# cfnptr/garden

Measured on AMD Instinct MI355X. Metric: entity culls/sec at 10M entities; visible-set bit-match vs CPU ref, higher is better.
Workload: dtype f32; 1 GPU; cfg3: 10M entities, frustum + Hi-Z occlusion vs synthetic 4096^2 depth pyramid (rebuilt per frame); depth=walls, entities_per_gpu=10000000, entities_total=10000000, scaling_mode=weak: 10000000 entities per GPU, hiz=4096x4096, prewarm_frames=2800

## Files before the change

### garden_amd/csrc/gv_cull.hip

```cpp
#include "gv_device.hpp"

#include <type_traits>

namespace gv {

template <typename F>
__host__ __device__ __forceinline__ void with_mapping(uint32_t mapping, F&& f)
{
    switch (mapping) {
    case kMapExact: f(std::integral_constant<uint32_t, kMapExact>{}); break;
    case kMapSpeculate: f(std::integral_constant<uint32_t, kMapSpeculate>{}); break;
    default: f(std::integral_constant<uint32_t, kMapGeneral>{}); break;
    }
}
template <typename F>
__host__ __device__ __forceinline__ void with_variant(bool hiz, uint32_t mapping, F&& f)
{
    if (hiz)
        with_mapping(mapping, [&](auto map) { f(std::true_type{}, map); });
    else
        with_mapping(mapping, [&](auto map) { f(std::false_type{}, map); });
}

__device__ __forceinline__ bool block_behind_planes(const float4 lo, const float4 hi, const float (&planes)[6][4],
                                                    uint32_t plane_count, const float (&cam)[3], uint32_t max_depth)
{
    const float mag = fmaxf(fabsf(lo.x), fabsf(hi.x)) + fmaxf(fabsf(lo.y), fabsf(hi.y)) + fmaxf(fabsf(lo.z), fabsf(hi.z)) +
                      fabsf(cam[0]) + fabsf(cam[1]) + fabsf(cam[2]);
    const float margin = 0.01f + 4e-5f * (float)(max_depth + 1u) * mag;
    bool behind = false;
#pragma unroll
    for (uint32_t p = 0; p < 6; p++)
        if (p < plane_count) {
            const float nx = planes[p][0], ny = planes[p][1], nz = planes[p][2];
            const float x = (nx >= 0.0f ? hi.x : lo.x) - cam[0];
            const float y = (ny >= 0.0f ? hi.y : lo.y) - cam[1];
            const float z = (nz >= 0.0f ? hi.z : lo.z) - cam[2];
            const float d = fmaf(nx, x, fmaf(ny, y, fmaf(nz, z, planes[p][3])));
            behind = behind || (d < -fmaf(4e-5f, fabsf(planes[p][3]), margin));
        }
    return behind;
}

typedef const CullArgs __attribute__((address_space(4))) * ConstCullArgs;
__device__ __forceinline__ void reload_cull_args(CullArgs& out)
{
    ConstCullArgs kernarg = (ConstCullArgs)__builtin_amdgcn_kernarg_segment_ptr();
    asm volatile("" : "+s"(kernarg));
    __builtin_memcpy(&out, kernarg, sizeof(out));
}

template <bool HIZ, uint32_t MAP, bool RELOAD = false, bool HOT = false>
__device__ __forceinline__ void cull_block(const CullArgs& args0, uint32_t lb, uint32_t* wave_count)
{
    static_assert(!HOT || MAP == kMapExact, "the sphere stream exists for exactly paired pools only");
    CullArgs stage1;
    if (RELOAD)
        reload_cull_args(stage1);
    const CullArgs& args = RELOAD ? stage1 : args0;
    uint32_t tid = threadIdx.x;
    if (RELOAD)
        asm volatile("" : "+v"(tid));
    const uint32_t i = lb * kCullBlock + tid;
    const uint32_t lane = tid & 63u, wave = tid >> 6;
    bool visible = false;
    Corners c;
    if (HOT && i < args.mesh.count) {
        const float4 h = stream_load(&args.mesh.hot[i]);
        uint32_t where = kSphereOutside;
        if (!(h.w < 0.0f)) {
            const float tx = h.x - args.view.cam[0], ty = h.y - args.view.cam[1], tz = h.z - args.view.cam[2];
            where = classify_sphere(tx, ty, tz, sphere_reach(h.w, tx, ty, tz), args.view.planes, args.view.plane_count);
        }
        visible = where == kSphereInside;
        if (where == kSphereUndecided || (HIZ && visible)) {
            Mat34 m;
            float4 box_a;
            float2 box_b;
            visible = prepare_model<MAP>(args.mesh, args.xf, args.view.cam, i, m, box_a, box_b) &&
                      settle<HIZ>(where, m, box_a, box_b, args.view.planes, args.view.plane_count, c);
        }
    } else if (!HOT && i < args.mesh.count) {
        Mat34 m;
        float4 box_a;
        float2 box_b;
        uint32_t where = kSphereOutside;
        if (prepare_model<MAP>(args.mesh, args.xf, args.view.cam, i, m, box_a, box_b))
            where = classify_sphere(m, box_a, box_b, args.view.planes, args.view.plane_count);
        visible = settle<HIZ>(where, m, box_a, box_b, args.view.planes, args.view.plane_count, c);
    }
    if (HIZ && visible) {
        CullArgs stage2;
        if (RELOAD)
            reload_cull_args(stage2);
        const CullArgs& a2 = RELOAD ? stage2 : args0;
        visible = !hiz_occluded(a2.hiz, a2.view.vp, c);
    }
    CullArgs stage3;
    if (RELOAD)
        reload_cull_args(stage3);
    const CullArgs& out_args = RELOAD ? stage3 : args0;
    if (i < out_args.mesh.count && out_args.view.write_is_visible)
        out_args.out.is_visible[i] = visible ? 1 : 0;
    __shared__ unsigned long long wave_word[kCullBlock / 64];
    const unsigned long long word = __ballot(visible);
    if (lane == 0) {
        wave_word[wave] = word;
        wave_count[wave] = (uint32_t)__popcll(word);
    }
    __syncthreads();
    if (tid < kCullBlock / 64)
        out_args.out.mask[(size_t)lb * (kCullBlock / 64) + tid] = wave_word[tid];
    if (tid == 0) {
        uint32_t total = 0;
#pragma unroll
        for (uint32_t w = 0; w < kCullBlock / 64; w++)
            total += wave_count[w];
        if (total)
            atomicAdd(&out_args.out.chunk_count[lb / (kEmitChunk / kCullBlock)], total);
    }
}

template <bool HIZ, uint32_t MAP, bool HOT = false>
__global__ __launch_bounds__(kCullBlock) void cull_kernel(const CullArgs args)
{
    __shared__ uint32_t wave_count[kCullBlock / 64];
    const uint32_t lb = tile_of_workgroup(blockIdx.x, args.xcd_run);
    if (lb >= args.nblocks)
        return;
    cull_block<HIZ, MAP, false, HOT>(args, lb, wave_count);
}

template <bool HIZ, uint32_t K>
__global__ __launch_bounds__(kCullBlock) void cull_hot_kernel(const CullArgs args)
{
    static_assert(K >= 2 && K <= 16 && (kEmitChunk / kCullBlock) % K == 0, "a super-tile must not straddle an emit chunk");
    __shared__ unsigned long long words[K * (kCullBlock / 64)];
    __shared__ uint32_t wave_count[kCullBlock / 64];
    const uint32_t first = tile_of_workgroup(blockIdx.x, args.xcd_run) * K;
    if (first >= args.nblocks)
        return;
    const uint32_t tid = threadIdx.x, lane = tid & 63u, wave = tid >> 6;
    const uint32_t base = first * kCullBlock + tid;
    float4 h[K];
#pragma unroll
    for (uint32_t k = 0; k < K; k++) {
        const uint32_t i = base + k * kCullBlock;
        h[k] = i < args.mesh.count ? stream_load(&args.mesh.hot[i]) : make_float4(0.0f, 0.0f, 0.0f, kHotDropped);
    }
    uint32_t where = 0;
#pragma unroll
    for (uint32_t k = 0; k < K; k++)
        if (!(h[k].w < 0.0f)) {
            const float tx = h[k].x - args.view.cam[0], ty = h[k].y - args.view.cam[1], tz = h[k].z - args.view.cam[2];
            where |= classify_sphere(tx, ty, tz, sphere_reach(h[k].w, tx, ty, tz), args.view.planes, args.view.plane_count) << (2u * k);
        }
    uint32_t count = 0;
#pragma unroll 1
    for (uint32_t k = 0; k < K; k++) {
        const uint32_t i = base + k * kCullBlock;
        const uint32_t wk = (where >> (2u * k)) & 3u;
        bool visible = wk == kSphereInside;
        if (wk == kSphereUndecided || (HIZ && visible)) {
            CullArgs a1;
            reload_cull_args(a1);
            Mat34 m;
            float4 box_a;
            float2 box_b;
            Corners c;
            visible = prepare_model<kMapExact>(a1.mesh, a1.xf, a1.view.cam, i, m, box_a, box_b) &&
                      settle<HIZ>(wk, m, box_a, box_b, a1.view.planes, a1.view.plane_count, c);
            if (HIZ && visible) {
                CullArgs a2;
                reload_cull_args(a2);
                visible = !hiz_occluded(a2.hiz, a2.view.vp, c);
            }
        }
        CullArgs a3;
        reload_cull_args(a3);
        if (i < a3.mesh.count && a3.view.write_is_visible)
            a3.out.is_visible[i] = visible ? 1 : 0;
        const unsigned long long word = __ballot(visible);
        if (lane == 0) {
            words[k * (kCullBlock / 64) + wave] = word;
            count += (uint32_t)__popcll(word);
        }
    }
    if (lane == 0)
        wave_count[wave] = count;
    __syncthreads();
    if (tid < K * (kCullBlock / 64) && first + tid / (kCullBlock / 64) < args.nblocks)
        args.out.mask[(size_t)first * (kCullBlock / 64) + tid] = words[tid];
    if (tid == 0) {
        uint32_t total = 0;
#pragma unroll
        for (uint32_t w = 0; w < kCullBlock / 64; w++)
            total += wave_count[w];
        if (total)
            atomicAdd(&args.out.chunk_count[first / (kEmitChunk / kCullBlock)], total);
    }
}

struct BlockWindow {
    uint32_t block;
    uint32_t level;
    uint32_t origin;
    float znear;
};
__device__ __forceinline__ BlockWindow block_window(const HizDevice& hz, const ViewParams& view, const float4 lo, const float4 hi,
                                                    uint32_t max_depth, uint32_t lb)
{
    BlockWindow out{lb, 0xFFu, 0u, 0.0f};
    if (!hz.nested)
        return out;
    const float (&vp)[16] = view.vp;
    const float mag = fmaxf(fabsf(lo.x), fabsf(hi.x)) + fmaxf(fabsf(lo.y), fabsf(hi.y)) + fmaxf(fabsf(lo.z), fabsf(hi.z)) +
                      fabsf(view.cam[0]) + fabsf(view.cam[1]) + fabsf(view.cam[2]);
    const float margin = 0.01f + 4e-5f * (float)(max_depth + 1u) * mag;
    const float bx[2] = {lo.x - view.cam[0] - margin, hi.x - view.cam[0] + margin};
    const float by[2] = {lo.y - view.cam[1] - margin, hi.y - view.cam[1] + margin};
    const float bz[2] = {lo.z - view.cam[2] - margin, hi.z - view.cam[2] + margin};
    const float inf = __builtin_huge_valf();
    float nx0 = inf, nx1 = -inf, ny0 = inf, ny1 = -inf, znear = -inf, wmin = inf;
    bool bounded = true;
#pragma unroll
    for (int k = 0; k < 8; k++) {
        const float x = bx[k & 1], y = by[(k >> 1) & 1], z = bz[k >> 2];
        const float clx = fmaf(vp[0], x, fmaf(vp[4], y, fmaf(vp[8], z, vp[12])));
        const float cly = fmaf(vp[1], x, fmaf(vp[5], y, fmaf(vp[9], z, vp[13])));
        const float clz = fmaf(vp[2], x, fmaf(vp[6], y, fmaf(vp[10], z, vp[14])));
        const float clw = fmaf(vp[3], x, fmaf(vp[7], y, fmaf(vp[11], z, vp[15])));
        bounded = bounded && (clw > 0.0f);
        const float rcp = 1.0f / clw;
        const float ndx = clx * rcp, ndy = cly * rcp, ndz = clz * rcp;
        nx0 = fminf(nx0, ndx); nx1 = fmaxf(nx1, ndx);
        ny0 = fminf(ny0, ndy); ny1 = fmaxf(ny1, ndy);
        znear = fmaxf(znear, ndz);
        wmin = fminf(wmin, clw);
    }
    if (!bounded)
        return out;
    const float r = lo.w;
    const float r0 = fmaxf(fmaxf(fabsf(vp[0]), fabsf(vp[4])), fabsf(vp[8])), r1 = fmaxf(fmaxf(fabsf(vp[1]), fabsf(vp[5])), fabsf(vp[9]));
    const float r3 = fmaxf(fmaxf(fabsf(vp[3]), fabsf(vp[7])), fabsf(vp[11]));
    const float span = 2.0f * r / wmin;
    const float ext_x = 0.5f * (float)hz.width * span * fmaf(fmaxf(fabsf(nx0), fabsf(nx1)), r3, r0) + 3.0f;
    const float ext_y = 0.5f * (float)hz.height * span * fmaf(fmaxf(fabsf(ny0), fabsf(ny1)), r3, r1) + 3.0f;
    const float n_max = fmaxf(ext_x, ext_y);
    if (!(n_max < 32768.0f))
        return out;
    const uint32_t l_max = (31u - (uint32_t)__clz((int)n_max)) + 1u;
    const int W = (int)hz.width, H = (int)hz.height;
    const float umin = clamp01(fmaf(nx0, 0.5f, 0.5f)), umax = clamp01(fmaf(nx1, 0.5f, 0.5f));
    const float vmin = clamp01(fmaf(ny0, 0.5f, 0.5f)), vmax = clamp01(fmaf(ny1, 0.5f, 0.5f));
    const int ix0 = max((int)(umin * (float)W) - 1, 0), ix1 = min((int)(umax * (float)W) + 1, W - 1);
    const int iy0 = max((int)(vmin * (float)H) - 1, 0), iy1 = min((int)(vmax * (float)H) + 1, H - 1);
    uint32_t level = min(l_max, hz.mip_count - 1u);
    while (level + 1u < hz.mip_count && (((ix1 >> level) - (ix0 >> level)) > 15 || ((iy1 >> level) - (iy0 >> level)) > 15))
        level++;
    const int lw = max(W >> level, 1), lh = max(H >> level, 1);
    const int tx0 = min(ix0 >> level, lw - 1), tx1 = min(ix1 >> level, lw - 1);
    const int ty0 = min(iy0 >> level, lh - 1), ty1 = min(iy1 >> level, lh - 1);
    if (tx1 - tx0 > 15 || ty1 - ty0 > 15)
        return out;
    out.level = level | ((uint32_t)(tx1 - tx0) << 8) | ((uint32_t)(ty1 - ty0) << 12);
    out.origin = (uint32_t)tx0 | ((uint32_t)ty0 << 16);
    out.znear = fmaf(fabsf(znear), 2e-6f, znear);
    return out;
}

struct ClassifyArgs {
    BlockBounds bounds;
    HizDevice hiz;
    ViewParams view;
    unsigned long long* mask;
    uint8_t* is_visible;
    uint32_t* kept_count;
    BlockWindow* kept;
    uint8_t* kept_flag;
    uint32_t nblocks, count, max_depth;
};

__device__ __forceinline__ void write_skipped_block(const ClassifyArgs& a, uint32_t lb)
{
    uint4* words = reinterpret_cast<uint4*>(a.mask + (size_t)lb * (kCullBlock / 64));
    words[0] = make_uint4(0, 0, 0, 0);
    words[1] = make_uint4(0, 0, 0, 0);
    if (a.view.write_is_visible) {
        const uint32_t first = lb * kCullBlock, end = min(first + kCullBlock, a.count);
        for (uint32_t s = first; s < end; s++)
            a.is_visible[s] = 0;
    }
}

template <bool HIZ>
__global__ __launch_bounds__(64) void block_classify_kernel(const ClassifyArgs a)
{
    const uint32_t lb = blockIdx.x * 64u + threadIdx.x;
    bool kept = false;
    BlockWindow win{lb, 0xFFu, 0u, 0.0f};
    if (lb < a.nblocks) {
        const float4 lo = a.bounds.lo[lb], hi = a.bounds.hi[lb];
        kept = !(lo.x > hi.x || block_behind_planes(lo, hi, a.view.planes, a.view.plane_count, a.view.cam, a.max_depth));
        if (HIZ && kept)
            win = block_window(a.hiz, a.view, lo, hi, a.max_depth, lb);
        if (!HIZ || !kept)
            a.bounds.examined[lb] = kept ? 1 : 0;
        if (!kept)
            write_skipped_block(a, lb);
    }
    const unsigned long long keep = __ballot(kept);
    if (keep == 0ull)
        return;
    uint32_t base = 0;
    if (threadIdx.x == 0)
        base = atomicAdd(a.kept_count, (uint32_t)__popcll(keep));
    base = (uint32_t)__builtin_amdgcn_readfirstlane((int)base);
    if (kept)
        a.kept[base + (uint32_t)__popcll(keep & ((1ull << threadIdx.x) - 1ull))] = win;
}

__global__ __launch_bounds__(256) void block_window_kernel(const ClassifyArgs a)
{
    const uint32_t lane = threadIdx.x & 63u;
    const uint32_t waves = gridDim.x * 4u;
    const uint32_t first = (uint32_t)__builtin_amdgcn_readfirstlane((int)(blockIdx.x * 4u + (threadIdx.x >> 6)));
    BlockWindow next = a.kept[min(first, a.nblocks - 1u)];
    const uint32_t listed = *a.kept_count;
    const float inf = __builtin_huge_valf();
    for (uint32_t j = first; j < listed; j += waves) {
        const BlockWindow w = next;
        if (j + waves < listed)
            next = a.kept[j + waves];
        bool occluded = false;
        const uint32_t level = w.level & 0xFFu;
        if (level != 0xFFu) {
            const uint32_t dx = (w.level >> 8) & 15u, dy = (w.level >> 12) & 15u, tx0 = w.origin & 0xFFFFu, ty0 = w.origin >> 16;
            const uint32_t lw = max(a.hiz.width >> level, 1u);
            const uint32_t lx = lane & 15u;
            float m = inf;
            bool nan = false;
#pragma unroll
            for (uint32_t q = 0; q < 4; q++) {
                const uint32_t ly = (lane >> 4) + 4u * q;
                float t = inf;
                if (lx <= dx && ly <= dy)
                    t = hiz_min_texel(a.hiz, level, lw, tx0 + lx, ty0 + ly);
                nan = nan || t != t;
                m = fminf(m, t);
            }
#pragma unroll
            for (uint32_t d = 32; d >= 1; d >>= 1)
                m = fminf(m, __shfl_xor(m, d, 64));
            occluded = __ballot(nan) == 0ull && w.znear < m;
        }
        if (lane == 0) {
            a.kept_flag[j] = occluded ? 0 : 1;
            a.bounds.examined[w.block] = occluded ? 0 : 1;
        }
        if (occluded) {
            if (lane < kCullBlock / 64)
                a.mask[(size_t)w.block * (kCullBlock / 64) + lane] = 0ull;
            if (a.view.write_is_visible) {
                const uint32_t slot = w.block * kCullBlock + 4u * lane;
                if (slot + 3u < a.count)
                    *reinterpret_cast<uint32_t*>(a.is_visible + slot) = 0u;
                else
                    for (uint32_t s = 0; slot + s < a.count && s < 4u; s++)
                        a.is_visible[slot + s] = 0;
            }
        }
    }
}

struct CullListArgs {
    const uint32_t* kept_count;
    const BlockWindow* kept;
    const uint8_t* kept_flag;
    uint32_t* next_count;
};

template <bool HIZ, uint32_t MAP>
__global__ __launch_bounds__(kCullBlock, 8) void cull_list_kernel(const CullArgs args, const CullListArgs la)
{
    __shared__ uint32_t wave_count[kCullBlock / 64];
    uint32_t flag = la.kept_flag ? la.kept_flag[blockIdx.x] : 1u;
    uint32_t block = la.kept[blockIdx.x].block;
    const uint32_t listed = *la.kept_count;
    if (blockIdx.x == 0 && threadIdx.x == 0)
        *la.next_count = 0;
    for (uint32_t j = blockIdx.x; j < listed;) {
        if (__builtin_amdgcn_readfirstlane((int)flag)) {
            cull_block<HIZ, MAP, true>(args, (uint32_t)__builtin_amdgcn_readfirstlane((int)block), wave_count);
            __syncthreads();
        }
        j += gridDim.x;
        if (j < listed) {
            flag = la.kept_flag ? la.kept_flag[j] : 1u;
            block = la.kept[j].block;
        }
    }
}

hipError_t launch_cull_listed(const MeshMirror& mesh, const TransformMirror& xf, const HizDevice& hiz, const ViewParams& vp,
                              const ViewBuffers& out, const BlockBounds& bounds, uint32_t* kept_count, uint32_t* next_count,
                              void* kept_list, uint8_t* kept_flag, hipStream_t stream)
{
    if (mesh.count == 0)
        return hipSuccess;
    const uint32_t nblocks = (mesh.count + kCullBlock - 1) / kCullBlock;
    const bool window_test = vp.use_hiz && hiz.nested;
    ClassifyArgs c{};
    c.bounds = bounds;
    c.hiz = hiz;
    c.view = vp;
    c.mask = out.mask;
    c.is_visible = out.is_visible;
    c.kept_count = kept_count;
    c.kept = static_cast<BlockWindow*>(kept_list);
    c.kept_flag = kept_flag;
    c.nblocks = nblocks;
    c.count = mesh.count;
    c.max_depth = xf.max_depth;
    const uint32_t list_grid = (nblocks + 3u) / 4u;
    if (window_test) {
        hipLaunchKernelGGL(block_classify_kernel<true>, dim3((nblocks + 63) / 64), dim3(64), 0, stream, c);
        hipLaunchKernelGGL(block_window_kernel, dim3((list_grid + 3u) / 4u), dim3(256), 0, stream, c);
    } else {
        hipLaunchKernelGGL(block_classify_kernel<false>, dim3((nblocks + 63) / 64), dim3(64), 0, stream, c);
    }
    CullArgs a{};
    a.mesh = mesh;
    a.xf = xf;
    a.hiz = hiz;
    a.view = vp;
    a.out = out;
    a.nblocks = nblocks;
    const CullListArgs la{kept_count, static_cast<const BlockWindow*>(kept_list), window_test ? kept_flag : nullptr, next_count};
    with_variant(vp.use_hiz, mesh.mapping, [&](auto hiz, auto map) {
        hipLaunchKernelGGL((cull_list_kernel<hiz, map>), dim3(list_grid), dim3(kCullBlock), 0, stream, a, la);
    });
    return hipGetLastError();
}
size_t cull_list_entry_bytes() { return sizeof(BlockWindow); }

struct FusedEmit {
    unsigned long long* status;
    uint32_t* ticket;
    uint32_t ticket_base;
    uint32_t epoch;
};
constexpr unsigned long long kTileAggregate = 1ull << 30, kTilePrefix = 2ull << 30, kTileFlagMask = 3ull << 30, kTileCountMask = (1ull << 30) - 1ull;

template <bool HIZ, uint32_t MAP>
__global__ __launch_bounds__(kCullBlock) void cull_emit_kernel(const CullArgs args, const FusedEmit fe)
{
    __shared__ uint32_t wave_count[kCullBlock / 64];
    __shared__ uint32_t tile_s, base_s;
    __shared__ float4 stage[kCullBlock * 3];
// ... 1197 lines not shown
```

### garden_amd/csrc/gv_device.hpp

```cpp
#pragma once
#include "gv_kernels.hpp"

#include <algorithm>

#include "gv_device_math.hpp"

namespace gv {


typedef float f32x4n __attribute__((ext_vector_type(4)));
typedef float f32x2n __attribute__((ext_vector_type(2)));
__device__ __forceinline__ float4 stream_load(const float4* p)
{
    const f32x4n v = __builtin_nontemporal_load(reinterpret_cast<const f32x4n*>(p));
    return make_float4(v.x, v.y, v.z, v.w);
}
__device__ __forceinline__ float2 stream_load(const float2* p)
{
    const f32x2n v = __builtin_nontemporal_load(reinterpret_cast<const f32x2n*>(p));
    return make_float2(v.x, v.y);
}
__device__ __forceinline__ uint32_t stream_load(const uint32_t* p) { return __builtin_nontemporal_load(p); }
__device__ __forceinline__ void stream_store(float4* p, float4 v)
{
    __builtin_nontemporal_store(f32x4n{v.x, v.y, v.z, v.w}, reinterpret_cast<f32x4n*>(p));
}
__device__ __forceinline__ void stream_store(float* p, float v) { __builtin_nontemporal_store(v, p); }
__device__ __forceinline__ uint32_t stream_load(const uint8_t* p) { return __builtin_nontemporal_load(p); }

struct XfRecord {
    float4 a, b;
    float2 c;
    uint32_t flags;
};
__device__ __forceinline__ XfRecord load_xf(const TransformMirror& xf, uint32_t s)
{
    XfRecord r;
    r.a = xf.ab[s].a;
    r.b = xf.ab[s].b;
    r.c = xf.c[s];
    r.flags = xf.flags[s];
    return r;
}
__device__ __forceinline__ XfRecord gather_xf(const TransformMirror& xf, uint32_t s, bool with_flags)
{
    XfRecord r;
    r.a = xf.ab[s].a;
    r.b = xf.ab[s].b;
    r.c = xf.c[s];
    r.flags = with_flags ? xf.flags[s] : 0u;
    return r;
}
__device__ __forceinline__ XfRecord stream_xf(const TransformMirror& xf, uint32_t s)
{
    XfRecord r;
    r.a = stream_load(&xf.ab[s].a);
    r.b = stream_load(&xf.ab[s].b);
    r.c = stream_load(&xf.c[s]);
    r.flags = stream_load(&xf.flags[s]);
    return r;
}
__device__ __forceinline__ Mat34 local_model(const XfRecord& r)
{
    return calc_model(r.a.x, r.a.y, r.a.z, r.b.x, r.b.y, r.b.z, r.b.w, r.a.w, r.c.x, r.c.y);
}

__device__ __forceinline__ void model_rows(const Mat34& m, float4& w0, float4& w1, float4& w2)
{
    w0 = make_float4(m.c0x, m.c0y, m.c0z, m.c1x);
    w1 = make_float4(m.c1y, m.c1z, m.c2x, m.c2y);
    w2 = make_float4(m.c2z, m.c3x, m.c3y, m.c3z);
}
__device__ __forceinline__ Mat34 rows_model(const float4 w0, const float4 w1, const float4 w2)
{
    Mat34 m;
    m.c0x = w0.x; m.c0y = w0.y; m.c0z = w0.z;
    m.c1x = w0.w; m.c1y = w1.x; m.c1z = w1.y;
    m.c2x = w1.z; m.c2y = w1.w; m.c2z = w2.x;
    m.c3x = w2.y; m.c3y = w2.z; m.c3z = w2.w;
    return m;
}

__device__ __forceinline__ Mat34 chain_model(const TransformMirror& xf, Mat34 m, uint32_t s, uint32_t flags)
{
    if (xf.max_depth != 0 && (flags & kXfWithAncestors)) {
        uint32_t p = xf.parent[s];
        for (uint32_t d = 0; d < xf.max_depth && p != kSlotNone; d++) {
            const XfRecord pr = load_xf(xf, p);
            m = mul_affine(local_model(pr), m);
            p = xf.parent[p];
        }
    }
    return m;
}

__device__ __forceinline__ float hiz_min_texel(const HizDevice& hz, uint32_t level, uint32_t lw, uint32_t x, uint32_t y)
{
    if (level == 0)
        return hz.depth[(size_t)y * hz.width + x];
    if (level == 1 && hz.level1_virtual) {
        const float2* row0 = reinterpret_cast<const float2*>(hz.depth + (size_t)(2 * y) * hz.width + 2 * x);
        const float2* row1 = reinterpret_cast<const float2*>(hz.depth + (size_t)(2 * y + 1) * hz.width + 2 * x);
        const float2 a = *row0, b = *row1;
        float m = a.x;
        m = a.y < m ? a.y : m;
        m = b.x < m ? b.x : m;
        m = b.y < m ? b.y : m;
        return hz.rg16f ? half_to_float(half_directed(m, false)) : m;
    }
    const uint64_t at = hz.mip_offset[level] + (uint64_t)y * lw + x;
    if (hz.rg16f)
        return half_to_float(reinterpret_cast<const uint32_t*>(hz.mips)[at] & 0xFFFFu);
    return hz.mips[at].x;
}
__device__ __forceinline__ float2 hiz_pair(const HizDevice& hz, uint64_t at)
{
    if (hz.rg16f)
        return unpack_rg16f(reinterpret_cast<const uint32_t*>(hz.mips)[at]);
    return hz.mips[at];
}

__device__ __forceinline__ float clamp01(float a)
{
    return a > 0.0f ? (a < 1.0f ? a : 1.0f) : 0.0f;
}

constexpr uint32_t kHizCoarseStep = 4;

__device__ __forceinline__ bool hiz_occluded(const HizDevice& hz, const float (&vp)[16], const Corners& c)
{
    float u[8], v[8], zc[8];
    bool bounded = true;
#pragma unroll
    for (int j = 0; j < 4; j++) {
        const v2f clx = pk_fma(splat(vp[0]), c.x[j], pk_fma(splat(vp[4]), c.y[j], pk_fma(splat(vp[8]), c.z[j], splat(vp[12]))));
        const v2f cly = pk_fma(splat(vp[1]), c.x[j], pk_fma(splat(vp[5]), c.y[j], pk_fma(splat(vp[9]), c.z[j], splat(vp[13]))));
        const v2f clz = pk_fma(splat(vp[2]), c.x[j], pk_fma(splat(vp[6]), c.y[j], pk_fma(splat(vp[10]), c.z[j], splat(vp[14]))));
        const v2f clw = pk_fma(splat(vp[3]), c.x[j], pk_fma(splat(vp[7]), c.y[j], pk_fma(splat(vp[11]), c.z[j], splat(vp[15]))));
        bounded = bounded && (clw.x > 0.0f) && (clw.y > 0.0f);
        const v2f rcp = {1.0f / clw.x, 1.0f / clw.y};
        const v2f uu = pk_fma(clx * rcp, splat(0.5f), splat(0.5f));
        const v2f vv = pk_fma(cly * rcp, splat(0.5f), splat(0.5f));
        const v2f zz = clz * rcp;
        u[2 * j] = uu.x; u[2 * j + 1] = uu.y;
        v[2 * j] = vv.x; v[2 * j + 1] = vv.y;
        zc[2 * j] = zz.x; zc[2 * j + 1] = zz.y;
    }
    if (!bounded)
        return false;
    const float umin0 = fminf(fminf(fminf(u[0], u[1]), fminf(u[2], u[3])), fminf(fminf(u[4], u[5]), fminf(u[6], u[7])));
    const float umax0 = fmaxf(fmaxf(fmaxf(u[0], u[1]), fmaxf(u[2], u[3])), fmaxf(fmaxf(u[4], u[5]), fmaxf(u[6], u[7])));
    const float vmin0 = fminf(fminf(fminf(v[0], v[1]), fminf(v[2], v[3])), fminf(fminf(v[4], v[5]), fminf(v[6], v[7])));
    const float vmax0 = fmaxf(fmaxf(fmaxf(v[0], v[1]), fmaxf(v[2], v[3])), fmaxf(fmaxf(v[4], v[5]), fmaxf(v[6], v[7])));
    const float znear = fmaxf(fmaxf(fmaxf(zc[0], zc[1]), fmaxf(zc[2], zc[3])), fmaxf(fmaxf(zc[4], zc[5]), fmaxf(zc[6], zc[7])));
    float umin = umin0, umax = umax0, vmin = vmin0, vmax = vmax0;
    umin = clamp01(umin);
    umax = clamp01(umax);
    vmin = clamp01(vmin);
    vmax = clamp01(vmax);
    const int W = (int)hz.width, H = (int)hz.height;
    int ix0 = (int)(umin * (float)W), ix1 = (int)(umax * (float)W);
    int iy0 = (int)(vmin * (float)H), iy1 = (int)(vmax * (float)H);
    ix0 = min(ix0, W - 1);
    ix1 = min(ix1, W - 1);
    iy0 = min(iy0, H - 1);
    iy1 = min(iy1, H - 1);
    auto axis_level = [](int i0, int i1) -> uint32_t {
        const int n = i1 - i0;
        if (n <= 1)
            return 0u;
        const uint32_t l = 31u - (uint32_t)__clz(n);
        return ((i1 >> l) - (i0 >> l)) <= 1 ? l : l + 1u;
    };
    const uint32_t level = min(max(axis_level(ix0, ix1), axis_level(iy0, iy1)), hz.mip_count - 1u);
    if (hz.nested && level + kHizCoarseStep < hz.mip_count) {
        const uint32_t cl = level + kHizCoarseStep;
        const int cw = max((int)(hz.width >> cl), 1), ch = max((int)(hz.height >> cl), 1);
        const int cx0 = min(ix0 >> cl, cw - 1), cx1 = min(ix1 >> cl, cw - 1);
        const int cy0 = min(iy0 >> cl, ch - 1), cy1 = min(iy1 >> cl, ch - 1);
        const uint64_t coarse = hz.mip_offset[cl];
        float2 t = hiz_pair(hz, coarse + (uint64_t)cy0 * cw + cx0);
        float cmin = t.x, cmax = t.y;
        if (cx1 != cx0) {
            t = hiz_pair(hz, coarse + (uint64_t)cy0 * cw + cx1);
            cmin = fminf(cmin, t.x);
            cmax = fmaxf(cmax, t.y);
        }
        if (cy1 != cy0) {
            t = hiz_pair(hz, coarse + (uint64_t)cy1 * cw + cx0);
            cmin = fminf(cmin, t.x);
            cmax = fmaxf(cmax, t.y);
            if (cx1 != cx0) {
                t = hiz_pair(hz, coarse + (uint64_t)cy1 * cw + cx1);
                cmin = fminf(cmin, t.x);
                cmax = fmaxf(cmax, t.y);
            }
        }
        if (znear < cmin)
            return true;
        if (znear >= cmax)
            return false;
    }
    const int lw = max((int)(hz.width >> level), 1), lh = max((int)(hz.height >> level), 1);
    const int tx0 = min(ix0 >> level, lw - 1), tx1 = min(ix1 >> level, lw - 1);
    const int ty0 = min(iy0 >> level, lh - 1), ty1 = min(iy1 >> level, lh - 1);
    float zfar = hiz_min_texel(hz, level, lw, tx0, ty0);
    float a = hiz_min_texel(hz, level, lw, tx1, ty0);
    zfar = a < zfar ? a : zfar;
    a = hiz_min_texel(hz, level, lw, tx0, ty1);
    zfar = a < zfar ? a : zfar;
    a = hiz_min_texel(hz, level, lw, tx1, ty1);
    zfar = a < zfar ? a : zfar;
    return znear < zfar;
}

inline uint32_t xcd_run_for_tiles(uint32_t tiles)
{
    return tiles >= 8u * 256u * 8u ? 256u : (tiles >= 8u * 32u * 8u ? 32u : 0u);
}

__device__ __forceinline__ uint32_t tile_of_workgroup(uint32_t b, uint32_t run)
{
    if (run == 0)
        return b;
    const uint32_t xcd = b & 7u, k = b >> 3;
    return ((k / run) * 8u + xcd) * run + k % run;
}

inline uint32_t grid_for_tiles(uint32_t tiles, uint32_t run)
{
    const uint32_t group = run * 8u;
    return run ? (tiles + group - 1) / group * group : tiles;
}

struct CullArgs {
    MeshMirror mesh;
    TransformMirror xf;
    HizDevice hiz;
    ViewParams view;
    ViewBuffers out;
    uint32_t nblocks;
    uint32_t xcd_run;
};

__device__ __forceinline__ bool mesh_entry_dropped(bool candidate, const float4& a, const float2& b, uint32_t xf_flags)
{
    const bool empty = (a.w - a.x <= 0.0f) && (b.x - a.y <= 0.0f) && (b.y - a.z <= 0.0f);
    return !candidate || empty || !(xf_flags & kXfActive);
}

template <uint32_t MAP>
__device__ __forceinline__ bool prepare_model(const MeshMirror& mesh, const TransformMirror& xf, const float (&cam)[3],
                                              uint32_t i, Mat34& m, float4& ma, float2& mb)
{
    ma = stream_load(&mesh.a[i]);
    mb = stream_load(&mesh.b[i]);
    uint32_t slot = i;
    bool candidate = true;
    XfRecord r = {};
    if (MAP == kMapGeneral) {
        const uint32_t link = stream_load(&mesh.link[i]);
        slot = link & kSlotMask;
        candidate = (link & kMeshCandidate) && slot != kSlotNone;
        if (candidate)
            r = load_xf(xf, slot);
    } else {
        const bool own = i < xf.count;
        if (own) {
            if (MAP == kMapExact && xf.max_depth == 0) {
                r.a = stream_load(&xf.ab[i].a);
                r.b = stream_load(&xf.ab[i].b);
                r.c = stream_load(&xf.c[i]);
                r.flags = (uint32_t)((xf.active_bits[i >> 6] >> (i & 63u)) & 1ull) * kXfActive;
            } else {
                r = stream_xf(xf, i);
            }
        }
        if (MAP == kMapSpeculate) {
            const uint32_t link = stream_load(&mesh.link[i]);
            slot = link & kSlotMask;
            candidate = (link & kMeshCandidate) && slot != kSlotNone;
            if (candidate && !(own && slot == i))
                r = load_xf(xf, slot);
        } else {
            candidate = own;
        }
    }
    if (mesh_entry_dropped(candidate, ma, mb, r.flags))
        return false;
    const Mat34 world = chain_model(xf, local_model(r), slot, r.flags);
    m = translated(world, cam[0], cam[1], cam[2]);
    return true;
}

__device__ __forceinline__ void aabb_corners(const Mat34& m, const float4 a, const float2 b, Corners& c)
{
    aabb_corners(m, a.x, a.y, a.z, a.w, b.x, b.y, c);
}

enum : uint32_t { kSphereOutside = 0, kSphereInside = 1, kSphereUndecided = 2 };
__device__ __forceinline__ float sphere_radius(const Mat34& m, const float4 a, const float2 b)
{
    const float ax = max_nan(fabsf(a.x), fabsf(a.w)), ay = max_nan(fabsf(a.y), fabsf(b.x)), az = max_nan(fabsf(a.z), fabsf(b.y));
    return fmaf(fabsf(m.c0x) + fabsf(m.c0y) + fabsf(m.c0z), ax,
                fmaf(fabsf(m.c1x) + fabsf(m.c1y) + fabsf(m.c1z), ay, (fabsf(m.c2x) + fabsf(m.c2y) + fabsf(m.c2z)) * az));
}
__device__ __forceinline__ float sphere_reach(float r, float tx, float ty, float tz)
{
    const float mag = max_nan(max_nan(fabsf(tx), fabsf(ty)), fabsf(tz)) + r;
    return fmaf(4e-5f, mag, r) + 0.01f;
}
__device__ __forceinline__ float sphere_reach(const Mat34& m, const float4 a, const float2 b)
{
    return sphere_reach(sphere_radius(m, a, b), m.c3x, m.c3y, m.c3z);
}
__device__ __forceinline__ uint32_t classify_sphere(float tx, float ty, float tz, float reach, const float (&planes)[6][4], uint32_t plane_count)
{
    bool outside = false, decided = true;
#pragma unroll
    for (uint32_t p = 0; p < 6; p++)
        if (p < plane_count) {
            const float bound = fmaf(4e-5f, fabsf(planes[p][3]), reach);
            const float d = fmaf(planes[p][0], tx, fmaf(planes[p][1], ty, fmaf(planes[p][2], tz, planes[p][3])));
            outside = outside | (d < -bound);
            decided = decided & ((d > bound) | (d < -bound));
        }
    return outside ? kSphereOutside : (decided ? kSphereInside : kSphereUndecided);
}
__device__ __forceinline__ uint32_t classify_sphere(const Mat34& m, float reach, const float (&planes)[6][4], uint32_t plane_count)
{
    return classify_sphere(m.c3x, m.c3y, m.c3z, reach, planes, plane_count);
}
__device__ __forceinline__ uint32_t classify_sphere(const Mat34& m, const float4 a, const float2 b, const float (&planes)[6][4],
                                                    uint32_t plane_count)
{
    return classify_sphere(m, sphere_reach(m, a, b), planes, plane_count);
}

__device__ __forceinline__ float4 hot_entry(const MeshMirror& mesh, const TransformMirror& xf, uint32_t i)
{
    const float zero[3] = {0.0f, 0.0f, 0.0f};
    Mat34 m;
    float4 a;
    float2 b;
    if (!prepare_model<kMapExact>(mesh, xf, zero, i, m, a, b))
        return make_float4(0.0f, 0.0f, 0.0f, kHotDropped);
    return make_float4(m.c3x, m.c3y, m.c3z, sphere_radius(m, a, b));
}

__device__ __forceinline__ bool behind_frustum(const Corners& c, const float (&planes)[6][4], uint32_t plane_count)
{
    bool behind = false;
#pragma unroll
    for (uint32_t p = 0; p < 6; p++)
        if (p < plane_count)
            behind = behind || all_behind_plane(c, planes[p][0], planes[p][1], planes[p][2], planes[p][3]);
    return behind;
}

template <bool HIZ>
__device__ __forceinline__ bool settle(uint32_t where, const Mat34& m, const float4 a, const float2 b, const float (&planes)[6][4],
                                       uint32_t plane_count, Corners& c)
{
    bool visible = where == kSphereInside;
    if (where == kSphereUndecided) {
        aabb_corners(m, a, b, c);
        visible = !behind_frustum(c, planes, plane_count);
    } else if (HIZ && visible) {
        aabb_corners(m, a, b, c);
    }
    return visible;
}
__device__ __forceinline__ bool settle(uint32_t where, bool hiz, const Mat34& m, const float4 a, const float2 b,
                                       const float (&planes)[6][4], uint32_t plane_count, Corners& c, bool& have_corners)
{
    bool visible = where == kSphereInside;
    if (where == kSphereUndecided || (hiz && visible)) {
        if (!have_corners) {
            aabb_corners(m, a, b, c);
            have_corners = true;
        }
        if (where == kSphereUndecided)
            visible = !behind_frustum(c, planes, plane_count);
    }
    return visible;
}

__device__ __forceinline__ float record_distance(const ViewParams& view, const Mat34& m)
{
    const float tx = m.c3x + view.cam_offset[0];
    const float ty = m.c3y + view.cam_offset[1];
    const float tz = m.c3z + view.cam_offset[2];
    return view.distance_2d ? m.c3z + 1.0f : fmaf(tz, tz, fmaf(ty, ty, tx * tx));
}
__device__ __forceinline__ void put_record(const ViewParams& view, const ViewBuffers& out, size_t rank, uint32_t slot, const Mat34& m,
                                           float4* row)
{
    out.visible_idx[rank] = slot;
    out.distance_sq[rank] = record_distance(view, m);
    model_rows(m, row[0], row[1], row[2]);
}
__device__ __forceinline__ void copy_rows(const float4* stage, float4* dst, uint32_t quads)
{
    for (uint32_t q = threadIdx.x; q < quads; q += 256)
        dst[q] = stage[q];
}

}
```

Before: 99.36 billion entity culls/s.

## Add conservative sphere-level Hi-Z occlusion pre-test before full box cull

```diff
diff --git a/garden_amd/csrc/gv_cull.hip b/garden_amd/csrc/gv_cull.hip
--- a/garden_amd/csrc/gv_cull.hip
+++ b/garden_amd/csrc/gv_cull.hip
@@ -70,7 +70,10 @@
         uint32_t where = kSphereOutside;
         if (!(h.w < 0.0f)) {
             const float tx = h.x - args.view.cam[0], ty = h.y - args.view.cam[1], tz = h.z - args.view.cam[2];
-            where = classify_sphere(tx, ty, tz, sphere_reach(h.w, tx, ty, tz), args.view.planes, args.view.plane_count);
+            const float reach = sphere_reach(h.w, tx, ty, tz);
+            where = classify_sphere(tx, ty, tz, reach, args.view.planes, args.view.plane_count);
+            if (HIZ && where != kSphereOutside && hiz_sphere_occluded(args.hiz, args.view.vp, tx, ty, tz, reach))
+                where = kSphereOutside;
         }
         visible = where == kSphereInside;
         if (where == kSphereUndecided || (HIZ && visible)) {
@@ -150,11 +153,36 @@
     }
     uint32_t where = 0;
 #pragma unroll
-    for (uint32_t k = 0; k < K; k++)
-        if (!(h[k].w < 0.0f)) {
+    for (uint32_t k = 0; k < K; k++) {
+        const bool kept = !(h[k].w < 0.0f);
+        if (kept || HIZ) {
             const float tx = h[k].x - args.view.cam[0], ty = h[k].y - args.view.cam[1], tz = h[k].z - args.view.cam[2];
-            where |= classify_sphere(tx, ty, tz, sphere_reach(h[k].w, tx, ty, tz), args.view.planes, args.view.plane_count) << (2u * k);
-        }
+            const float reach = sphere_reach(h[k].w, tx, ty, tz);
+            if (HIZ)
+                h[k] = make_float4(tx, ty, tz, reach);
+            if (kept)
+                where |= classify_sphere(tx, ty, tz, reach, args.view.planes, args.view.plane_count) << (2u * k);
+        }
+    }
+    if (HIZ && hiz_sphere_usable(args.hiz) && where != 0u) {
+#pragma unroll
+        for (uint32_t g = 0; g < K; g += 2) {
+            HizSphereQuery q[2];
+            float texel[2][4];
+#pragma unroll
+            for (uint32_t k = 0; k < 2; k++) {
+                q[k] = hiz_sphere_query(args.hiz, args.view.vp, h[g + k].x, h[g + k].y, h[g + k].z, h[g + k].w);
+                hiz_sphere_fetch(args.hiz, q[k], texel[k]);
+            }
+#pragma unroll
+            for (uint32_t k = 0; k < 2; k++)
+                if (hiz_sphere_proven(q[k], texel[k]))
+                    where &= ~(3u << (2u * (g + k)));
+            if (g + 2 < K)
+                asm volatile("" : "+v"(where), "+v"(h[(g + 2) % K].x), "+v"(h[(g + 2) % K].y), "+v"(h[(g + 2) % K].z), "+v"(h[(g + 2) % K].w),
+                             "+v"(h[(g + 3) % K].x), "+v"(h[(g + 3) % K].y), "+v"(h[(g + 3) % K].z), "+v"(h[(g + 3) % K].w));
+        }
+    }
     uint32_t count = 0;
 #pragma unroll 1
     for (uint32_t k = 0; k < K; k++) {
diff --git a/garden_amd/csrc/gv_device.hpp b/garden_amd/csrc/gv_device.hpp
--- a/garden_amd/csrc/gv_device.hpp
+++ b/garden_amd/csrc/gv_device.hpp
@@ -214,6 +214,83 @@
     return znear < zfar;
 }
 
+constexpr uint32_t kHizSphereStep = 2;
+struct HizSphereQuery {
+    float znear;
+    uint32_t at[4];
+};
+__device__ __forceinline__ bool hiz_sphere_usable(const HizDevice& hz)
+{
+    return hz.nested && hz.mip_count > 2u;
+}
+__device__ __forceinline__ HizSphereQuery hiz_sphere_query(const HizDevice& hz, const float (&vp)[16], float tx, float ty, float tz, float reach)
+{
+    const float cx = fmaf(vp[0], tx, fmaf(vp[4], ty, fmaf(vp[8], tz, vp[12])));
+    const float cy = fmaf(vp[1], tx, fmaf(vp[5], ty, fmaf(vp[9], tz, vp[13])));
+    const float cz = fmaf(vp[2], tx, fmaf(vp[6], ty, fmaf(vp[10], tz, vp[14])));
+    const float cw = fmaf(vp[3], tx, fmaf(vp[7], ty, fmaf(vp[11], tz, vp[15])));
+    const float ex = reach * (fabsf(vp[0]) + fabsf(vp[4]) + fabsf(vp[8]));
+    const float ey = reach * (fabsf(vp[1]) + fabsf(vp[5]) + fabsf(vp[9]));
+    const float ez = reach * (fabsf(vp[2]) + fabsf(vp[6]) + fabsf(vp[10]));
+    const float ew = reach * (fabsf(vp[3]) + fabsf(vp[7]) + fabsf(vp[11]));
+    const float wlo = cw - ew, whi = cw + ew;
+    const float rlo = 1.0f / wlo, rhi = 1.0f / whi;
+    const float xlo = cx - ex, xhi = cx + ex, ylo = cy - ey, yhi = cy + ey, zhi = cz + ez;
+    const float nx0 = xlo * (xlo >= 0.0f ? rhi : rlo), nx1 = xhi * (xhi >= 0.0f ? rlo : rhi);
+    const float ny0 = ylo * (ylo >= 0.0f ? rhi : rlo), ny1 = yhi * (yhi >= 0.0f ? rlo : rhi);
+    const float znear0 = zhi * (zhi >= 0.0f ? rlo : rhi);
+    const float probe = fabsf(nx0) + fabsf(nx1) + fabsf(ny0) + fabsf(ny1) + fabsf(znear0) + whi;
+    const bool bounded = (wlo > 0.0f) & (probe < __builtin_huge_valf());
+    HizSphereQuery q;
+    q.znear = bounded ? fmaf(fabsf(znear0), 2e-6f, znear0) : __builtin_nanf("");
+    const int W = (int)hz.width, H = (int)hz.height;
+    const float umin = clamp01(fmaf(nx0, 0.5f, 0.5f)), umax = clamp01(fmaf(nx1, 0.5f, 0.5f));
+    const float vmin = clamp01(fmaf(ny0, 0.5f, 0.5f)), vmax = clamp01(fmaf(ny1, 0.5f, 0.5f));
+    const int ix0 = max((int)(umin * (float)W) - 1, 0), ix1 = min((int)(umax * (float)W) + 1, W - 1);
+    const int iy0 = max((int)(vmin * (float)H) - 1, 0), iy1 = min((int)(vmax * (float)H) + 1, H - 1);
+    auto axis_level = [](int i0, int i1) -> uint32_t {
+        const int n = i1 - i0;
+        if (n <= 1)
+            return 0u;
+        const uint32_t l = 31u - (uint32_t)__clz(n);
+        return ((i1 >> l) - (i0 >> l)) <= 1 ? l : l + 1u;
+    };
+    const uint32_t cl = min(max(axis_level(ix0, ix1), axis_level(iy0, iy1)) + kHizSphereStep, hz.mip_count - 1u);
+    const int lw = max((int)(hz.width >> cl), 1), lh = max((int)(hz.height >> cl), 1);
+    const int x0 = min(ix0 >> cl, lw - 1), x1 = min(ix1 >> cl, lw - 1);
+    const int y0 = min(iy0 >> cl, lh - 1), y1 = min(iy1 >> cl, lh - 1);
+    const uint32_t first = (uint32_t)hz.mip_offset[cl];
+    q.at[0] = first + (uint32_t)(y0 * lw + x0);
+    q.at[1] = first + (uint32_t)(y0 * lw + x1);
+    q.at[2] = first + (uint32_t)(y1 * lw + x0);
+    q.at[3] = first + (uint32_t)(y1 * lw + x1);
+    return q;
+}
+__device__ __forceinline__ float hiz_stored_min(const HizDevice& hz, uint32_t at)
+{
+    const uint32_t word = reinterpret_cast<const uint32_t*>(hz.mips)[hz.rg16f ? at : 2u * at];
+    return hz.rg16f ? half_to_float(word & 0xFFFFu) : __uint_as_float(word);
+}
+__device__ __forceinline__ void hiz_sphere_fetch(const HizDevice& hz, const HizSphereQuery& q, float (&t)[4])
+{
+#pragma unroll
+    for (int j = 0; j < 4; j++)
+        t[j] = hiz_stored_min(hz, q.at[j]);
+}
+__device__ __forceinline__ bool hiz_sphere_proven(const HizSphereQuery& q, const float (&t)[4])
+{
+    return (q.znear < t[0]) & (q.znear < t[1]) & (q.znear < t[2]) & (q.znear < t[3]);
+}
+__device__ __forceinline__ bool hiz_sphere_occluded(const HizDevice& hz, const float (&vp)[16], float tx, float ty, float tz, float reach)
+{
+    if (!hiz_sphere_usable(hz))
+        return false;
+    const HizSphereQuery q = hiz_sphere_query(hz, vp, tx, ty, tz, reach);
+    float t[4];
+    hiz_sphere_fetch(hz, q, t);
+    return hiz_sphere_proven(q, t);
+}
+
 inline uint32_t xcd_run_for_tiles(uint32_t tiles)
 {
     return tiles >= 8u * 256u * 8u ? 256u : (tiles >= 8u * 32u * 8u ? 32u : 0u);
```

Result: faster. 106.0 billion entity culls/s, median of 6 (+6.7%).
